# loganmcbroom/Flan

Measured on AMD Instinct MI355X. Metric: PV analysis+resynthesis frames/sec (2048-win, hop 512, 48 kHz) at 1/2/4/8 GPU, higher is better.
Workload: dtype f32; 1 GPU; 8 ch x 60 s x 48 kHz uniform noise per GPU, convert_to_PV(2048,512,dft 2048) -> convert_to_audio round trip; channels_per_gpu=8, parallelism=channel-shard x1

## Files before the change

### flan_amd/__init__.py

```python
import ctypes as C
import os

import numpy as np

_HERE = os.path.dirname(os.path.abspath(__file__))
LIB_PATH = os.environ.get("FLAN_AMD_LIB") or os.path.join(_HERE, "libflanhip.so")

OK, ERR_INVALID_ARG, ERR_UNSUPPORTED, ERR_HIP, ERR_CANCELLED, ERR_NO_DEVICE = 0, -1, -2, -3, -4, -5


class FlanHipError(RuntimeError):
    def __init__(self, code, message):
        super().__init__("flanhip error %d: %s" % (code, message))
        self.code = code


if not os.path.exists(LIB_PATH):
    raise ImportError("flan_amd/libflanhip.so is missing: build it with `python flan_amd/build.py` "
                      "(hipcc --offload-arch=gfx950); there is no fallback path")

lib = C.CDLL(LIB_PATH)

_f32p = np.ctypeslib.ndpointer(np.float32, flags="C_CONTIGUOUS")
_vp, _i64, _i32, _f32 = C.c_void_p, C.c_int64, C.c_int, C.c_float
# ... 13 lines not shown
    "flanhip_download": (C.c_int, [_vp, _vp, C.c_size_t]),
    "flanhip_touch_pages": (C.c_int, [_vp, C.c_size_t]),
    "flanhip_host_workers": (C.c_int, []),
    "flanhip_parallel_for": (C.c_int, [C.c_int, _vp, _vp]),
    "flanhip_stream_create": (C.c_int, [C.POINTER(_vp)]),
    "flanhip_stream_destroy": (C.c_int, [_vp]),
    "flanhip_host_malloc": (C.c_int, [C.POINTER(_vp), C.c_size_t]),
    "flanhip_host_free": (C.c_int, [_vp]),
    "flanhip_memcpy_h2d": (C.c_int, [_vp, _vp, C.c_size_t, _vp]),
    "flanhip_memcpy_d2h": (C.c_int, [_vp, _vp, C.c_size_t, _vp]),
    "flanhip_memset": (C.c_int, [_vp, _i32, C.c_size_t, _vp]),
    "flanhip_stream_synchronize": (C.c_int, [_vp]),
    "flanhip_wait_cancellable": (C.c_int, [_vp, _vp]),
    "flanhip_wait_cancellable_fn": (C.c_int, [_vp, _vp, _vp]),
    "flanhip_analyze": (C.c_int, [_vp, _i64, _i64, _f32, _i32, _i32, _i32, _vp, C.POINTER(_i64), _vp]),
    "flanhip_analyze_dev": (C.c_int, [_vp, _i64, _i64, _f32, _i32, _i32, _i32, _vp, _vp]),
    "flanhip_synthesize": (C.c_int, [_vp, _i64, _i64, _i32, _f32, _f32, _i32, _vp, C.POINTER(_i32), _vp]),
    "flanhip_synthesize_workspace_bytes": (C.c_size_t, [_i64, _i64, _i32, _f32, _f32, _i32]),
    "flanhip_synthesize_dev": (C.c_int, [_vp, _i64, _i64, _i32, _f32, _f32, _i32, _vp, _vp, _vp, _vp]),
    "flanhip_analyze_dev_fused": (C.c_int, [_vp, _i64, _i64, _f32, _i32, _i32, _i32, _vp, _vp, _vp]),
    "flanhip_synthesize_dev_fused": (C.c_int, [_vp, _i64, _i64, _i32, _f32, _f32, _i32, _vp, _vp, _vp, _vp]),
    "flanhip_synthesize_dev_stages": (C.c_int, [_vp, _i64, _i64, _i32, _f32, _f32, _i32, _vp, _vp, _vp, _i32, _i32, _vp]),
    "flanhip_debug_option": (None, [_i32, _i32]),
    "flanhip_debug_kernel_scratch_bytes": (_i32, [_i32]),
    "flanhip_modify_time": (C.c_int, [_vp, _i64, _i64, _i32, _f32, _i32, _vp, _i64, _vp, _vp]),
    "flanhip_modify_time_dev": (C.c_int, [_vp, _i64, _i64, _i32, _f32, _i32, _vp, _i64, _vp, _vp]),
    "flanhip_modify_time_dev_fused": (C.c_int, [_vp, _i64, _i64, _i32, _f32, _f32, _vp, _i64, _vp, _i32, _vp, _vp]),
    "flanhip_synthesize_dev_fused_checked": (C.c_int, [_vp, _i64, _i64, _i32, _f32, _f32, _i32, _vp, _vp, _vp, _vp]),
    "flanhip_stretch_map_dev": (C.c_int, [_vp, _i64, _i32, _f32, _i32, _vp, _vp]),
    "flanhip_stretch_map_const_dev": (C.c_int, [_f32, _vp, _i64, _i32, _f32, _i32, _vp, _vp]),
    "flanhip_fill_dev": (C.c_int, [_vp, _i64, _f32, _vp]),
    "flanhip_modify_frequency": (C.c_int, [_vp, _i64, _i64, _i32, _f32, _vp, _vp, _vp, _vp]),
    "flanhip_modify_frequency_dev": (C.c_int, [_vp, _i64, _i64, _i32, _f32, _vp, _vp, _vp, _vp]),
    "flanhip_modify_time_interp_dev": (C.c_int, [_vp, _i64, _i64, _i32, _f32, _i32, _vp, _i64, _i32, _vp, _vp]),
    "flanhip_modify_time_interp_dev_fused": (C.c_int, [_vp, _i64, _i64, _i32, _f32, _f32, _vp, _i64, _i32, _vp, _i32, _vp, _vp]),
    "flanhip_modify_frequency_interp_dev": (C.c_int, [_vp, _i64, _i64, _i32, _f32, _vp, _vp, _i32, _vp, _vp]),
    "flanhip_repitch_interp_dev": (C.c_int, [_vp, _i64, _i64, _i32, _f32, _vp, _i32, _vp, _vp]),
    "flanhip_repitch_map_dev": (C.c_int, [_vp, _i64, _i64, _i32, _f32, _vp, _vp, _vp]),
    "flanhip_repitch_dev": (C.c_int, [_vp, _i64, _i64, _i32, _f32, _vp, _vp, _vp]),
    "flanhip_shape_affine": (C.c_int, [_vp, _i64, _i64, _i32, _f32, _f32, _f32, _f32, _f32, _i32, _vp, _vp]),
    "flanhip_shape_affine_dev": (C.c_int, [_vp, _i64, _i64, _i32, _f32, _f32, _f32, _f32, _f32, _i32, _vp, _vp]),
    "flanhip_shape_table_dev": (C.c_int, [_vp, _vp, _i64, _i64, _i32, _f32, _i32, _vp, _vp]),
    "flanhip_replace_amplitudes_dev": (C.c_int, [_vp, _i64, _i64, _i32, _vp, _i64, _i64, _i32, _vp, _f32, _vp, _vp]),
    "flanhip_subtract_amplitudes_dev": (C.c_int, [_vp, _i64, _i64, _i32, _vp, _i64, _i64, _i32, _vp, _f32, _vp, _vp]),
    "flanhip_resonate_out_frames": (_i64, [_i64, _f32, _f32, _i32]),
    "flanhip_resonate_dev": (C.c_int, [_vp, _i64, _i64, _i32, _f32, _i32, _i64, _vp, _f32, _vp, _vp]),
# ... 442 lines not shown


def analyze_dev(d_audio, ch, n, sample_rate, window, hop, dft, d_out, stream=None):
    check(lib.flanhip_analyze_dev(_dp(d_audio), ch, n, sample_rate, window, hop, dft, _dp(d_out), _vp(stream or 0)))


def analyze_dev_fused(d_audio, ch, n, sample_rate, window, hop, dft, d_out, d_ws, stream=None):
    check(lib.flanhip_analyze_dev_fused(_dp(d_audio), ch, n, sample_rate, window, hop, dft, _dp(d_out), _dp(d_ws), _vp(stream or 0)))


def synthesize_dev_fused(d_pv, ch, F, bins, sample_rate, analysis_rate, window, d_out, d_ws, d_nan=None, stream=None):
    check(lib.flanhip_synthesize_dev_fused(_dp(d_pv), ch, F, bins, sample_rate, analysis_rate, window, _dp(d_out), _dp(d_ws),
                                           _dp(d_nan), _vp(stream or 0)))


def synthesize_dev_stages(d_pv, ch, F, bins, sample_rate, analysis_rate, window, d_out, d_ws, d_nan, presummed, stages, stream=None):
    check(lib.flanhip_synthesize_dev_stages(_dp(d_pv), ch, F, bins, sample_rate, analysis_rate, window, _dp(d_out), _dp(d_ws),
                                            _dp(d_nan), presummed, stages, _vp(stream or 0)))


DEBUG_CHAIN_LEN, DEBUG_TARGET_CHAINS, DEBUG_FORCE_GENERIC, DEBUG_NO_FAST_DIV = 0, 1, 2, 3
DEBUG_ANA_VARIANT, DEBUG_SYN_VARIANT, DEBUG_ANA4096_OLD, DEBUG_SYN4096_OLD, DEBUG_RESAMPLE_DIRECT, DEBUG_FORCE_DIRECT, DEBUG_INLINE_FIXUP, DEBUG_WIDE_OFFSETS = 4, 5, 6, 7, 8, 9, 10, 11
_DEBUG_NAMES = {"chain_len": 0, "target_chains": 1, "force_generic": 2, "no_fast_div": 3, "ana_variant": 4, "syn_variant": 5,
                "ana4096_old": 6, "syn4096_old": 7, "resample_direct": 8, "force_direct": 9, "inline_fixup": 10, "wide_offsets": 11, "no_sub": 12}


class debug_options:

    def __init__(self, **kw):
        self.kw = {_DEBUG_NAMES[k]: int(v) for k, v in kw.items()}

    def __enter__(self):
        for k, v in self.kw.items():
            lib.flanhip_debug_option(k, v)
        return self

    def __exit__(self, *exc):
        for k in self.kw:
            lib.flanhip_debug_option(k, 0)
        return False


def synthesize_workspace_bytes(ch, F, bins, sample_rate, analysis_rate, window):
    return int(lib.flanhip_synthesize_workspace_bytes(ch, F, bins, sample_rate, analysis_rate, window))


def synthesize_dev(d_pv, ch, F, bins, sample_rate, analysis_rate, window, d_out, d_ws, d_nan=None, stream=None):
# ... 101 lines not shown
```

### flan_amd/csrc/conversions.hip

```cpp
#include "flanhip_internal.h"
#include <atomic>
#include <memory>
#include "pv_kernels.h"
#include "pv_kernels_fast.h"
#include <type_traits>
#include "pv_kernels_v2.h"
#include "pv_kernels_v3.h"
#include "pv_kernels_eo.h"
#include "pv_kernels_any.h"
#include "pv_kernels_mr.h"
#include "pv_kernels_bs.h"
#include "pv_kernels_big.h"
#include "team_launch.h"
#include "sub_launch.h"
#include <algorithm>
#include <cstdlib>

namespace flanhip {


static constexpr int kMaxAnyDft = 1 << 20;
static bool fft_size( int dft ) { return is_pow2( dft ) && dft >= 32 && dft <= 8192; }
static int mr_blocks_per_cu( const MrPlan & pl, int W )
	{
// ... 342 lines not shown
	const bool n_ok = n >= 2 && n < ( int64_t( 1 ) << 31 ) - 8192;
	route_pow2( r, dft, n_ok && sub_shape( dft, W, hop ),
		n_ok && ( dft == 2048 || ( dft == 4096 && !debug_options().ana11_old ) || v3_size( dft ) ) && hop <= 65536 && !force_generic() );
	return r;
	}
static Route synthesis_route( int dft, int W, int hop )
	{
	Route r = size_route( dft, W, hop );
	r.min_len = r.family == Family::any ? 1 : std::max( ( W + hop - 1 ) / hop - 1, 1 );
	if( r.family != Family::generic ) return r;
	const bool sub = sub_shape( dft, W, hop );
	r.kind = sub ? 0 : synth_fast_kind( dft, W, hop );
	route_pow2( r, dft, sub, r.kind != 0 );
	return r;
	}

static int self_carry_group( const Route & syn, const SynthLayout & lay )
	{
	if( syn.family != Family::sub && syn.family != Family::fast ) return 0;
	if( syn.family == Family::fast && lay.dft == 4096 && debug_options().ana11_old ) return 0;
	return lay.chains_per_channel < 128 ? 0 : syn.block_group;
	}
static int synth_layout_routed( int64_t ch, int64_t F, int bins, float sr, float ar, int W, SynthLayout * o, Route * route );
int synth_layout( int64_t ch, int64_t F, int bins, float sr, float ar, int W, SynthLayout * o ) { Route r; return synth_layout_routed( ch, F, bins, sr, ar, W, o, &r ); }

static int launch_group_scan( const SynthParams & p, hipStream_t s )
	{
	if( p.groups_per_channel <= 512 ) hipLaunchKernelGGL( ( k_phase_scan2<16, true> ), dim3( (unsigned) ( ( p.num_bins + 31 ) / 32 ), (unsigned) p.num_channels ), dim3( 512 ), 0, s, p );
	else hipLaunchKernelGGL( ( k_phase_scan2<32, true> ), dim3( (unsigned) ( ( p.num_bins + 15 ) / 16 ), (unsigned) p.num_channels ), dim3( 512 ), 0, s, p );
	FLANHIP_CHECK( hipGetLastError() );
	return FLANHIP_OK;
	}
static int launch_group_sums( bool sums_too, int gsize, const SynthParams & p, double * gs, hipStream_t s )
	{
	const dim3 grid( (unsigned) ( ( p.num_bins + 255 ) / 256 ), (unsigned) p.groups_per_channel, (unsigned) p.num_channels );
	auto kern = sums_too ? ( gsize == 32 ? k_sums_and_groups<32> : gsize == 16 ? k_sums_and_groups<16> : gsize == 8 ? k_sums_and_groups<8> : k_sums_and_groups<4> )
		: ( gsize == 32 ? k_group_sums<32> : gsize == 16 ? k_group_sums<16> : gsize == 8 ? k_group_sums<8> : k_group_sums<4> );
	hipLaunchKernelGGL( kern, grid, dim3( 256 ), 0, s, p, gs );
	FLANHIP_CHECK( hipGetLastError() );
	return FLANHIP_OK;
	}
template<bool B> using bool_c = std::integral_constant<bool, B>;
template<int I> using int_c = std::integral_constant<int, I>;
template<typename F> static auto mr_kernel( const MrPlan & pl, F f )
	{
	return !mr_pingpong( pl.C ) ? f( bool_c<false>{}, bool_c<true>{} ) : mr_plan_is_big( pl ) ? f( bool_c<true>{}, bool_c<true>{} ) : f( bool_c<true>{}, bool_c<false>{} );
	}
template<typename F> static auto bs_kernel( const BsPlan & pl, int W, F f )
	{
	return !bs_pingpong( pl.M ) ? f( bool_c<false>{}, bool_c<false>{} ) : bs_hoist( pl, W ) ? f( bool_c<true>{}, bool_c<true>{} ) : f( bool_c<true>{}, bool_c<false>{} );
	}
template<int MIXED, typename F> static auto big_kernel_q( int bq, F f ) { return bq > 4 ? f( int_c<8>{}, int_c<MIXED>{} ) : bq > 2 ? f( int_c<4>{}, int_c<MIXED>{} ) : f( int_c<2>{}, int_c<MIXED>{} ); }
template<typename F> static auto big_kernel( const BigPlan & pl, F f )
	{
	const int bq = ( pl.C2 + MR_THREADS - 1 ) / MR_THREADS;
	return pl.mixed == 2 ? big_kernel_q<2>( bq, f ) : pl.mixed ? big_kernel_q<1>( bq, f ) : big_kernel_q<0>( bq, f );
	}

static int launch_analyze_body( const float * d_audio, int64_t ch, int64_t n, float sr, int W, int hop, int dft, flanhip_MF * d_out, void * d_fused_ws, hipStream_t s, bool * left_group_sums, int * epoch );

int launch_analyze( const float * d_audio, int64_t ch, int64_t n, float sr, int W, int hop, int dft, flanhip_MF * d_out, void * d_fused_ws, hipStream_t s )
	{
	bool left_group_sums = false;
	int epoch = 0;
	if( d_fused_ws ) note_workspace_producer( d_fused_ws, 0 );
	const int rc = launch_analyze_body( d_audio, ch, n, sr, W, hop, dft, d_out, d_fused_ws, s, &left_group_sums, &epoch );
	if( !rc && d_fused_ws && left_group_sums ) note_workspace_producer( d_fused_ws, 1, epoch );
	return rc;
	}

static int launch_analyze_body( const float * d_audio, int64_t ch, int64_t n, float sr, int W, int hop, int dft, flanhip_MF * d_out, void * d_fused_ws, hipStream_t s, bool * left_group_sums, int * epoch )
	{
	FLANHIP_REQUIRE( d_audio && d_out, FLANHIP_ERR_INVALID_ARG, "null buffer" );
	FLANHIP_REQUIRE( ch > 0 && n >= 0 && W >= 2 && hop >= 1 && sr > 0.0f, FLANHIP_ERR_INVALID_ARG, "bad sizes" );
	FLANHIP_REQUIRE( W <= dft, FLANHIP_ERR_INVALID_ARG, "window_size larger than dft_size" );
	FLANHIP_REQUIRE( dft_size_ok( dft ), FLANHIP_ERR_UNSUPPORTED, "dft_size must be even, at least 4 and at most 2^20" );
	if( int rc = require_device() ) return rc;
	const Route r = analysis_route( dft, W, hop, n );
	std::shared_ptr<const PlanRef> plan_ref;
	if( int rc = get_plan( W, dft, &plan_ref ) ) return rc;
	const Plan * plan = &plan_ref->plan;

	AnalyzeParams p{};
	p.audio = d_audio; p.out = reinterpret_cast<MF*>( d_out );
	p.window = plan->d_window; p.tw = plan->d_tw; p.tw2 = plan->d_tw2; p.dump = plan->d_dump;
	p.n = n; p.F = n / hop + 1;
	p.num_channels = int( ch ); p.window_size = W; p.hop = hop;
	p.L = choose_chain_length( ch, p.F, r.min_len, r.target_chains, r.block_group );
	p.chains_per_channel = int( ( p.F + p.L - 1 ) / p.L );
	p.sample_rate = sr;
	p.analysis_rate = sr / hop;
	DivPlan dp;
	if( int rc = get_div_plan( p.analysis_rate, &dp ) ) return rc;
	p.ar_div = DivC{ dp.c, dp.rc, dp.exact };
	p.sums = nullptr; p.nan_out = nullptr; p.nan_epoch = 0;
	p.cancel = thread_cancel_word( s );
	bool kernel_sums = r.family != Family::any && r.family != Family::big && ( r.family != Family::mr || mr_pingpong( r.mr.C ) ) && ( r.family != Family::bs || bs_pingpong( r.bs.M ) );
	SynthLayout fused_lay{};
	if( d_fused_ws )
		{
		SynthLayout & lay = fused_lay;
		Route syn;
		if( int rc = synth_layout_routed( ch, p.F, dft / 2 + 1, sr, p.analysis_rate, W, &lay, &syn ) ) return rc;
		p.nan_epoch = next_epoch();
		*epoch = p.nan_epoch;
		if( kernel_sums && lay.L >= p.L + 8 && int64_t( p.chains_per_channel ) * ch <= r.target_chains ) kernel_sums = false;
		if( kernel_sums )
			{
			p.L = lay.L;
			p.chains_per_channel = lay.chains_per_channel;
			p.sums = reinterpret_cast<double*>( d_fused_ws );
			p.nan_out = ws_at<int>( d_fused_ws, lay.carry_bytes + lay.head_bytes );
			}
		const bool groups_too = ( r.family == Family::fast || r.family == Family::sub ) && hop <= W && kernel_sums && self_carry_group( syn, lay ) != 0;
		p.group_sums = groups_too ? ws_at<double>( d_fused_ws, lay.group_offset ) : nullptr;
		p.groups_per_channel = lay.groups_per_channel;
		*left_group_sums = groups_too;
		}
	auto prepass_on_behalf = [&]() -> int
		{
		if( !d_fused_ws || kernel_sums ) return FLANHIP_OK;
		SynthParams q{};
		q.pv = reinterpret_cast<const MF*>( d_out );
		q.carry = reinterpret_cast<double*>( d_fused_ws );
		q.F = p.F; q.num_channels = int( ch ); q.num_bins = dft / 2 + 1;
		q.L = fused_lay.L; q.chains_per_channel = fused_lay.chains_per_channel;
		q.analysis_rate = p.analysis_rate; q.ar_div = p.ar_div;
		q.nan_words = ws_at<int>( d_fused_ws, fused_lay.carry_bytes + fused_lay.head_bytes );
		q.nan_epoch = p.nan_epoch;
		const int64_t chains = int64_t( q.chains_per_channel ) * ch;
		hipLaunchKernelGGL( k_phase_sums2, dim3( (unsigned) chains, (unsigned) ( ( q.num_bins + 255 ) / 256 ) ), dim3( 256 ), 0, s, q );
		FLANHIP_CHECK( hipGetLastError() );
		return FLANHIP_OK;
		};

	const int64_t chains = int64_t( p.chains_per_channel ) * ch;
	int rc = FLANHIP_ERR_UNSUPPORTED;
	switch( r.family )
		{
		case Family::team: rc = run_analyze_team( p, *plan, dft, s ); break;
// ... 167 lines not shown
	p.analysis_rate = ar;
	p.window_scale = 2.67f / ( lay.dft * W / lay.hop );
	DivPlan dp;
	if( int rc = get_div_plan( ar, &dp ) ) return rc;
	p.ar_div = DivC{ dp.c, dp.rc, dp.exact };
	p.dump = ws_at<float>( d_ws, lay.carry_bytes + lay.head_bytes + 512 );
	p.nan_in = ( presummed == 1 || presummed == 2 ) ? ws_at<const int>( d_ws, lay.carry_bytes + lay.head_bytes ) : nullptr;
	p.skip_words = presummed == 2 ? p.nan_in : nullptr;
	p.carry_in = d_carry_in; p.total_out = d_total_out; p.total_only = prepass_only ? 1 : 0;
	p.cancel = thread_cancel_word( s );
	const int fix_hook = debug_options().inline_fixup;
	const bool self_fix = lay.fix_offset != 0 && !prepass_only && ( stage_mask & 0xF ) == 0xF && fix_hook != 2
		&& ( fix_hook == 1 || lay.L >= ( lay.head_len + lay.hop - 1 ) / lay.hop + 3 );
	if( self_fix )
		{
		p.fix_state = ws_at<int>( d_ws, lay.fix_offset );
		p.tail = ws_at<float>( d_ws, lay.tail_offset );
		p.fix_tag = int( ( unsigned( next_epoch() ) & 0x1FFFFFFFu ) << 2 );
		}

	const int64_t chains = int64_t( p.chains_per_channel ) * ch;
	FLANHIP_REQUIRE( chains < ( int64_t( 1 ) << 31 ), FLANHIP_ERR_UNSUPPORTED, "too many chains for one launch" );
	const int stages = prepass_only ? 3 : ( stage_mask & 0xF );
	int noted_epoch = 0;
	const int gsize = self_carry_group( r, lay );
	const bool self_carry = presummed == 1 && !prepass_only && !d_carry_in && !d_total_out && debug_options().syn_variant != 2
		&& gsize != 0 && workspace_producer( d_ws, &noted_epoch ) == 1;
	if( self_carry )
		{
		p.expect_epoch = noted_epoch;
		p.group_sums = ws_at<const double>( d_ws, lay.group_offset );
		p.groups_per_channel = lay.groups_per_channel;
		const bool scan_groups = p.groups_per_channel > 40;
		p.group_carry = scan_groups ? ws_at<double>( d_ws, lay.group_offset + lay.group_bytes ) : nullptr;
		if( scan_groups && ( stages & 2 ) ) { if( int rc = launch_group_scan( p, s ) ) return rc; }
		}
	const bool group_kernel = !self_carry && gsize != 0 && stages == 0xF && !prepass_only && !d_carry_in && !d_total_out && debug_options().syn_variant != 2 && presummed != 3;
	const bool sums_in_group_kernel = group_kernel && presummed != 1;
	if( ( stages & 1 ) && presummed != 1 && presummed != 3 && !sums_in_group_kernel )
		{
		hipLaunchKernelGGL( k_phase_sums2, dim3( (unsigned) chains, (unsigned) ( ( bins + 255 ) / 256 ) ), dim3( 256 ), 0, s, p );
		FLANHIP_CHECK( hipGetLastError() );
		}
	if( group_kernel )
		{
		double * gs = ws_at<double>( d_ws, lay.group_offset );
		p.groups_per_channel = lay.groups_per_channel;
		FLANHIP_REQUIRE( lay.groups_per_channel <= 65535 && ch <= 65535, FLANHIP_ERR_UNSUPPORTED, "too many groups / channels for one launch" );
		if( int rc = launch_group_sums( sums_in_group_kernel, gsize, p, gs, s ) ) return rc;
		p.group_sums = gs;
		const bool scan_groups = p.groups_per_channel > 40;
		p.group_carry = scan_groups ? ws_at<double>( d_ws, lay.group_offset + lay.group_bytes ) : nullptr;
		if( scan_groups ) { if( int rc = launch_group_scan( p, s ) ) return rc; }
		}
	if( ( stages & 2 ) && !self_carry && !group_kernel )
		{
		const int64_t cols = ch * bins;
		const bool flat = p.chains_per_channel <= 64 && ( bins >= 2049 || cols >= 65536 ) && !d_carry_in && !d_total_out && !prepass_only;
		if( flat && p.chains_per_channel <= 32 ) hipLaunchKernelGGL( k_phase_scan_flat<32>, dim3( (unsigned) ( ( bins + 255 ) / 256 ), (unsigned) ch ), dim3( 256 ), 0, s, p );
		else if( flat ) hipLaunchKernelGGL( k_phase_scan_flat<64>, dim3( (unsigned) ( ( bins + 255 ) / 256 ), (unsigned) ch ), dim3( 256 ), 0, s, p );
		else if( p.chains_per_channel <= 512 ) hipLaunchKernelGGL( k_phase_scan2<16>, dim3( (unsigned) ( ( bins + 31 ) / 32 ), (unsigned) ch ), dim3( 512 ), 0, s, p );
		else if( p.chains_per_channel <= 1024 ) hipLaunchKernelGGL( k_phase_scan2<32>, dim3( (unsigned) ( ( bins + 15 ) / 16 ), (unsigned) ch ), dim3( 512 ), 0, s, p );
		else hipLaunchKernelGGL( k_phase_scan2<64>, dim3( (unsigned) ( ( bins + 7 ) / 8 ), (unsigned) ch ), dim3( 512 ), 0, s, p );
		FLANHIP_CHECK( hipGetLastError() );
		}

	int rc = FLANHIP_ERR_UNSUPPORTED;
	if( !( stages & 4 ) ) rc = FLANHIP_OK;
	else switch( r.family )
		{
		case Family::any:
			{
			std::shared_ptr<const UnitRef> unit_ref;
			if( int rc2 = get_unit_circle( lay.dft, &unit_ref ) ) return rc2;
// ... 178 lines not shown
	{
	FLANHIP_REQUIRE( presummed >= 0 && presummed <= 2, FLANHIP_ERR_INVALID_ARG, "presummed: 0, 1 or 2" );
	return launch_synthesize( d_pv, ch, F, bins, sr, ar, W, d_out, d_ws, d_nan, presummed, (hipStream_t) stream, nullptr, nullptr, false, stages );
	}

void flanhip_debug_option( int which, int value )
	{
	DebugOptions & o = debug_options();
	switch( which )
		{
		case FLANHIP_DEBUG_CHAIN_LEN:       o.chain_len = value; break;
		case FLANHIP_DEBUG_TARGET_CHAINS:   o.target_chains = value; break;
		case FLANHIP_DEBUG_FORCE_GENERIC:   o.force_generic = value; break;
		case FLANHIP_DEBUG_NO_FAST_DIV:     o.no_fast_div = value; break;
		case FLANHIP_DEBUG_ANA_VARIANT:     o.ana_variant = value; break;
		case FLANHIP_DEBUG_SYN_VARIANT:     o.syn_variant = value; break;
		case FLANHIP_DEBUG_ANA4096_OLD:     o.ana11_old = value; break;
		case FLANHIP_DEBUG_SYN4096_OLD:     o.syn11_old = value; break;
		case FLANHIP_DEBUG_RESAMPLE_DIRECT: o.resample_direct = value; break;
		case FLANHIP_DEBUG_FORCE_DIRECT:    o.force_direct = value; break;
		case FLANHIP_DEBUG_INLINE_FIXUP:    o.inline_fixup = value; break;
		case FLANHIP_DEBUG_WIDE_OFFSETS:    o.wide_offsets = value; break;
		case FLANHIP_DEBUG_NO_SUB:          o.no_sub = value; break;
		default: break;
		}
	}
#ifdef FLANHIP_STAMPS
int flanhip_debug_read_stamps( unsigned long long * out16 )
	{
	FLANHIP_CHECK( hipDeviceSynchronize() );
	FLANHIP_CHECK( hipMemcpyFromSymbol( out16, HIP_SYMBOL( g_stamp_acc ), 16 * sizeof( unsigned long long ) ) );
	unsigned long long zero[16] = { 0 };
	FLANHIP_CHECK( hipMemcpyToSymbol( HIP_SYMBOL( g_stamp_acc ), zero, sizeof( zero ) ) );
	return FLANHIP_OK;
	}
int flanhip_debug_read_spans( unsigned long long * out8192 )
	{
	FLANHIP_CHECK( hipDeviceSynchronize() );
	FLANHIP_CHECK( hipMemcpyFromSymbol( out8192, HIP_SYMBOL( g_stamp_span ), 8192 * sizeof( unsigned long long ) ) );
	return FLANHIP_OK;
	}
#endif

size_t flanhip_synthesize_workspace_bytes( int64_t ch, int64_t F, int bins, float sr, float ar, int W )
	{
	SynthLayout lay;
	if( synth_layout( ch, F, bins, sr, ar, W, &lay ) ) return 0;
	return lay.total_bytes;
	}

int flanhip_synthesize_dev( const flanhip_MF * d_pv, int64_t ch, int64_t F, int bins, float sr, float ar, int W,
	float * d_out, void * d_ws, int * d_nan, void * stream )
	{
	return launch_synthesize( d_pv, ch, F, bins, sr, ar, W, d_out, d_ws, d_nan, false, (hipStream_t) stream );
	}

int flanhip_synthesize( const flanhip_MF * pv, int64_t ch, int64_t F, int bins, float sr, float ar, int W,
	float * out, int * nan_flag, volatile int * cancel )
	{
	FLANHIP_REQUIRE( pv && out, FLANHIP_ERR_INVALID_ARG, "null buffer" );
	SynthLayout lay;
	if( int rc = synth_layout( ch, F, bins, sr, ar, W, &lay ) ) return rc;
	if( int rc = require_device() ) return rc;
	if( cancelled( cancel ) ) return FLANHIP_ERR_CANCELLED;
	const size_t pv_bytes = sizeof( flanhip_MF ) * size_t( ch ) * F * bins;
// ... 20 lines not shown
```

### flan_amd/csrc/flanhip_internal.h

```cpp
#pragma once
#include <hip/hip_runtime.h>
#include <cstdarg>
#include <cstdint>
#include <cstdio>
#include <cmath>
#include <map>
#include <memory>
#include <mutex>
#include <tuple>
#include <vector>

#include "flanhip.h"
#include "cf_type.h"

namespace flanhip {

void set_error( const char * fmt, ... );

#define FLANHIP_CHECK( expr )                                                                         \
	do { hipError_t e_ = ( expr );                                                                    \
		if( e_ != hipSuccess ) {                                                                      \
			::flanhip::set_error( "%s failed: %s (%s:%d)", #expr, hipGetErrorString( e_ ), __FILE__, __LINE__ ); \
			return FLANHIP_ERR_HIP; } } while( 0 )

// ... 37 lines not shown
	};
inline int team_radix( int dft_size ) { return dft_size == 8192 ? 4 : dft_size == 16384 ? 8 : 0; }
struct TeamTableLayout { int tw1, tw3, twj, tws, two, total; };
inline TeamTableLayout team_table_layout( int R ) { TeamTableLayout l; l.tw1 = 0; l.tw3 = 240; l.twj = 1008; l.tws = l.twj + ( R - 1 ) * 512; l.two = l.tws + ( R / 2 ) * 512; l.total = l.two + 2 * R; return l; }
struct PlanRef { Plan plan; PlanRef() = default; PlanRef( const PlanRef & ) = delete; PlanRef & operator=( const PlanRef & ) = delete; ~PlanRef(); };
int get_plan( int window_size, int dft_size, std::shared_ptr<const PlanRef> * out );

struct DivPlan { float c, rc; int exact; };
int get_div_plan( float c, DivPlan * out );

int choose_chain_length( int64_t num_channels, int64_t num_frames, int min_len, int target_chains, int group = 1 );
struct DebugOptions
	{
	int chain_len = 0;
	int target_chains = 0;
	int force_generic = 0;
	int no_fast_div = 0;
	int ana_variant = 0, syn_variant = 0;
	int ana11_old = 0, syn11_old = 0;
	int resample_direct = 0;
	int wide_offsets = 0;
	int inline_fixup = 0;
	int no_sub = 0;
	int force_direct = 0;
	};
DebugOptions & debug_options();
bool force_generic();
int cu_count();

int launch_analyze( const float * d_audio, int64_t ch, int64_t n, float sr, int W, int hop, int dft, flanhip_MF * d_out, void * d_fused_ws, hipStream_t s );
int launch_synthesize( const flanhip_MF * d_pv, int64_t ch, int64_t F, int bins, float sr, float ar, int W, float * d_out,
	void * d_ws, int * d_nan, int presummed, hipStream_t s, const double * d_carry_in = nullptr, double * d_total_out = nullptr,
	bool prepass_only = false, int stage_mask = 0xF );

int next_epoch();

struct SynthLayout { int hop, dft, L, chains_per_channel, head_len, groups_per_channel; size_t carry_bytes, head_bytes, group_offset, group_bytes, total_bytes;
	size_t flags_offset;
	size_t fix_offset, tail_offset;
	bool any; size_t any_spec_offset, any_frames_offset;
	size_t mr_ring_offset;
	size_t bsg_offset;
	bool big; size_t big_out_offset, big_head_offset, big_ring_offset; };
void note_workspace_producer( const void * d_ws, int kind, int epoch = 0 );
int workspace_producer( const void * d_ws, int * epoch = nullptr );
int synth_layout( int64_t ch, int64_t F, int bins, float sr, float ar, int W, SynthLayout * out );
// ... 9 lines not shown
```

### flan_amd/csrc/pv_kernels.h

```cpp
#pragma once
#include <hip/hip_runtime.h>
#include <stdint.h>
#include "fft_device.h"
#include "pv_math.h"

namespace flanhip {

struct MF { float m, f; };


struct AnalyzeParams
	{
	const float * audio;
	MF * out;
	const float * window;
	const cf * tw;
	const cf * tw2;
	int64_t n;
	int64_t F;
	int num_channels;
	int window_size;
	int hop;
	int L;
	int chains_per_channel;
	float sample_rate;
	float analysis_rate;
	DivC ar_div;
	double * sums;
	int * nan_out;
	int nan_epoch;
	double * group_sums;
	int groups_per_channel;
	const int * cancel;
	float * dump;
	};

__device__ __forceinline__ int cancel_peek( const int * word )
	{
	return word ? __hip_atomic_load( word, __ATOMIC_RELAXED, __HIP_MEMORY_SCOPE_SYSTEM ) : 0;
	}
__device__ __forceinline__ bool cancel_seen( int peeked ) { return __builtin_amdgcn_readfirstlane( peeked ) != 0; }

__device__ __forceinline__ MF phase_vocode_bin( float re, float im, float & prev_phase, float bin_frequency, float expected_phase_diff,
	float analysis_rate, bool use_wrapping )
	{
	const float phase = atan2_fast( im, re );
	const float phase_diff = phase - prev_phase;
	prev_phase = phase;
	const float delta_phase = phase_diff - expected_phase_diff;
	const float wrapped = use_wrapping ? delta_phase - FLANHIP_PI2_F * round_half_away( div_pi2( delta_phase ) ) : delta_phase;
	const float delta_frequency = div_pi2( wrapped * analysis_rate );
	MF r;
	r.m = magnitude_scaled( re, im );
	r.f = bin_frequency + delta_frequency;
	return r;
	}

// ... 194 lines not shown
	int chains_per_channel;
	int head_len;
	int num_bins;
	float analysis_rate;
	float window_scale;
	DivC ar_div;
	const int * nan_in;
	float * dump;
	const double * carry_in;
	double * total_out;
	int total_only;
	int * nan_words;
	int nan_epoch;
	int expect_epoch;
	const int * skip_words;
	const int * cancel;
	const double * group_sums;
	int groups_per_channel;
	double * group_carry;
	int * fix_state;
	float * tail;
	int fix_tag;
	float * ring_ws;
	};


template<int LOG2C, int WAVES, int T = 1>
__global__ __launch_bounds__( 64 * WAVES * T ) void k_synthesize( SynthParams p )
	{
	constexpr int C = 1 << LOG2C;
	static_assert( T == 1 || WAVES == 1, "a team of several wavefronts owns its block" );
	constexpr int TEAM = 64 * T, NT = 64 * WAVES * T;
	constexpr int E = ( C + TEAM - 1 ) / TEAM;
	constexpr bool BIG = LOG2C >= 12 && T == 1;
	constexpr int UNR = BIG ? 2 : E + 1;
	extern __shared__ __attribute__((aligned(16))) unsigned char smem[];
	cf * s_tw = reinterpret_cast<cf*>( smem );
	const int W = p.window_size, hop = p.hop;
	const int wpad = ( W + 3 ) & ~3;
	float * s_win = reinterpret_cast<float*>( s_tw + ( BIG ? 0 : C ) );
	cf * s_buf_all = reinterpret_cast<cf*>( s_win + wpad );
	float * s_ring_all = reinterpret_cast<float*>( s_buf_all + WAVES * padded_len( C + 1 ) );
	double * s_ph_all = reinterpret_cast<double*>( s_ring_all + WAVES * wpad );

	const int tid = threadIdx.x, lane = T == 1 ? ( tid & 63 ) : tid, wave = T == 1 ? ( tid >> 6 ) : 0;
	__shared__ int s_cancel;
// ... 200 lines not shown
```

### flan_amd/csrc/pv_kernels_v2.h

```cpp
#pragma once
#include "pv_kernels_fast.h"

namespace flanhip {

struct V2Lds
	{
	static constexpr int C = 1024;
	static constexpr int TW1 = 0;
	static constexpr int TW3 = TW1 + 240;
	static constexpr int W2H = TW3 + 768;
	static constexpr int WIN = W2H + 512;
	static constexpr int KC = WIN + 1024;
	static constexpr int BUF = KC + 1024;
	static constexpr int BUF_LEN = C + C / 16 + 1;
	static constexpr size_t bytes( int waves ) { return size_t( BUF + waves * BUF_LEN ) * 8; }
	};


#ifdef FLANHIP_STAMPS
__device__ unsigned long long g_stamp_acc[16];
__device__ unsigned long long g_stamp_span[2 * 4096];
struct Stamps
	{
	unsigned long long last, acc[12], t_begin, r_begin;
// ... 46 lines not shown
			const unsigned w = blockIdx.x * ( blockDim.x >> 6 ) + ( threadIdx.x >> 6 );
			if( w < 4096 ) { g_stamp_span[2 * w] = r_begin; g_stamp_span[2 * w + 1] = r_end; }
			}
		}
#endif
	};
#else
struct Stamps
	{
	__device__ __forceinline__ void init() {}
	__device__ __forceinline__ void operator()( int ) const {}
	__device__ __forceinline__ void flush( int ) {}
	};
#endif


#ifndef FLANHIP_PUBLISH_DRAIN
#define FLANHIP_PUBLISH_DRAIN 1
#endif
__device__ __forceinline__ void publish_drain()
	{
	if constexpr( FLANHIP_PUBLISH_DRAIN != 0 ) asm volatile( "s_waitcnt vmcnt(0)" ::: "memory" );
	else asm volatile( "" ::: "memory" );
	}

template<int WAVES, bool SUMS, int NV, int ABL = 0>
__global__ __launch_bounds__( 64 * WAVES ) void k_analyze_v2( AnalyzeParams p, FastTables tb )
	{
	using L = V2Lds;
	constexpr int C = 1024, E = 16, H = 8, NT = 64 * WAVES;
	constexpr int NP = NV / 2;
	static_assert( NV == 2 || NV == 4 || NV == 8 || NV == 16, "1, 2, 4 or 8 pairs at a time" );
	typedef float VB __attribute__(( ext_vector_type( NV ) ));
	extern __shared__ __attribute__((aligned(16))) unsigned char smem[];
	cf * s = reinterpret_cast<cf*>( smem );
	const int tid = threadIdx.x, lane = tid & 63, wave = tid >> 6;
	const int W = p.window_size, hop = p.hop;
	const int cancel_word = cancel_peek( p.cancel );

	for( int i = tid; i < 240; i += NT ) s[L::TW1 + i] = tb.tw1[i];
	for( int i = tid; i < 768; i += NT ) s[L::TW3 + i] = tb.tw3[i];
	for( int i = tid; i < 512; i += NT ) { const cf w = tb.w2[i]; s[L::W2H + i] = mk( 0.5f * w.x, 0.5f * w.y ); }
		{
		float * win = reinterpret_cast<float*>( s + L::WIN );
		for( int i = tid; i < 2 * C; i += NT ) win[i] = ( i < W ) ? p.window[i] : 0.0f;
		v4f_t * kc = reinterpret_cast<v4f_t*>( s + L::KC );
// ... 310 lines not shown
				}
			const double vx = fold( sumx );
			if( lane == 0 ) { dst[C / 2] = vx; stage[C / 2] = vx; }
			}
		const bool any_bad = __any( bad );
		if( p.nan_out && lane == 0 && active )
			{
			if( chain == 0 ) { p.nan_out[2] = p.nan_epoch; p.nan_out[4] = p.nan_epoch; }
			if( any_bad ) p.nan_out[0] = p.nan_epoch;
			}
		if( p.group_sums )
			{
			__syncthreads();
			const int live = min( WAVES, p.chains_per_channel - group * WAVES );
			double * gdst = p.group_sums + ( int64_t( channel ) * groups + group ) * ( C + 1 );
			for( int bin = tid; bin <= C; bin += NT )
				{
				double run = 0.0;
				for( int w = 0; w < live; ++w )
					{
					const double v = run + reinterpret_cast<const double*>( s + L::BUF + w * L::BUF_LEN )[bin];
					run = ( __builtin_fabs( v ) < FLANHIP_FOLD_FAST_LIMIT ) ? fold_phase_fast( v ) : fold_phase_any( v );
					}
				gdst[bin] = run;
				}
			}
		}
	}

__device__ __forceinline__ void st_agent( cf * p, cf v )
	{
	unsigned long long bits; __builtin_memcpy( &bits, &v, 8 );
	__hip_atomic_store( reinterpret_cast<unsigned long long*>( p ), bits, __ATOMIC_RELAXED, __HIP_MEMORY_SCOPE_AGENT );
	}
__device__ __forceinline__ cf ld_agent( const cf * p )
	{
	const unsigned long long bits = __hip_atomic_load( reinterpret_cast<const unsigned long long*>( p ), __ATOMIC_RELAXED, __HIP_MEMORY_SCOPE_AGENT );
	cf v; __builtin_memcpy( &v, &bits, 8 );
	return v;
	}

struct V2LdsSyn
	{
	static constexpr int C = 1024;
	static constexpr int TW1 = 0;
	static constexpr int TW3 = TW1 + 240;
	static constexpr int W2S = TW3 + 768;
// ... 141 lines not shown
			{
			#pragma unroll
			for( int b = 0; b < NB; ++b ) run[b] = gs[int64_t( group ) * ( C + 1 ) + bins_of[b]];
			}
		if( active ) load_row( relf0 );
		if( !p.group_carry )
			{
			for( int g0 = 0; g0 < group; g0 += 16 )
				{
				double v[NB][16];
				#pragma unroll
				for( int b = 0; b < NB; ++b )
					{
					#pragma unroll
					for( int u = 0; u < 16; ++u ) v[b][u] = ( g0 + u < group ) ? gs[int64_t( g0 + u ) * ( C + 1 ) + bins_of[b]] : 0.0;
					}
				#pragma unroll
				for( int u = 0; u < 16; ++u )
					{
					#pragma unroll
					for( int b = 0; b < NB; ++b ) run[b] = fold( run[b] + v[b][u] );
					}
				}
			}
		#pragma unroll
		for( int w = 0; w < WAVES; ++w )
			{
			#pragma unroll
			for( int b = 0; b < NB; ++b )
				{
				if( has[b] ) reinterpret_cast<double*>( s + L::BUF + w * L::BUF_LEN )[bins_of[b]] = run[b];
				run[b] = fold( run[b] + vc[b][w] );
				}
			}
		if( tid == 0 && blockIdx.x == 0 )
			{
			if( p.nan_in && p.nan_flag && p.nan_in[0] == p.nan_in[2] && p.nan_in[2] != 0 ) atomicOr( p.nan_flag, 1 );
			if( p.expect_epoch && p.nan_in && p.nan_flag && p.nan_in[2] != p.expect_epoch ) atomicOr( p.nan_flag, 2 );
			if( p.skip_words ) const_cast<int*>( p.skip_words )[4] = 0;
			}
		__syncthreads();
		const double * mine = reinterpret_cast<const double*>( buf );
		#pragma unroll
		for( int q = 0; q < H; ++q ) { phk[q] = mine[lane + 64 * q]; phm[q] = mine[C - lane - 64 * q]; }
		phx = mine[C / 2];
		wave_sync();
// ... 277 lines not shown
```

### include/flanhip.h

```cpp
#ifndef FLANHIP_H
#define FLANHIP_H

#include <stddef.h>
#include <stdint.h>

#ifdef __cplusplus
extern "C" {
#endif

#define FLANHIP_OK                 0
#define FLANHIP_ERR_INVALID_ARG   -1
#define FLANHIP_ERR_UNSUPPORTED   -2
#define FLANHIP_ERR_HIP           -3
#define FLANHIP_ERR_CANCELLED     -4
#define FLANHIP_ERR_NO_DEVICE     -5

typedef struct flanhip_MF { float m; float f; } flanhip_MF;

int          flanhip_version(void);
const char * flanhip_last_error(void);
int          flanhip_device_count(void);
int          flanhip_set_device(int device);
int          flanhip_get_device(int * device);

// ... 42 lines not shown
                                 float sample_rate, float analysis_rate, int window_size,
                                 float * d_out, void * d_workspace, int * d_nan_flag, void * stream);
int flanhip_synthesize_dev_fused_checked(const flanhip_MF * d_pv, int64_t num_channels, int64_t num_pv_frames, int num_bins,
                                         float sample_rate, float analysis_rate, int window_size,
                                         float * d_out, void * d_workspace, int * d_nan_flag, void * stream);

int flanhip_synthesize_dev_stages(const flanhip_MF * d_pv, int64_t num_channels, int64_t num_pv_frames, int num_bins,
                                  float sample_rate, float analysis_rate, int window_size,
                                  float * d_out, void * d_workspace, int * d_nan_flag, int presummed, int stages, void * stream);

#define FLANHIP_DEBUG_CHAIN_LEN       0
#define FLANHIP_DEBUG_TARGET_CHAINS   1
#define FLANHIP_DEBUG_FORCE_GENERIC   2
#define FLANHIP_DEBUG_NO_FAST_DIV     3
#define FLANHIP_DEBUG_ANA_VARIANT     4
#define FLANHIP_DEBUG_SYN_VARIANT     5
#define FLANHIP_DEBUG_ANA4096_OLD     6
#define FLANHIP_DEBUG_SYN4096_OLD     7
#define FLANHIP_DEBUG_RESAMPLE_DIRECT 8
#define FLANHIP_DEBUG_FORCE_DIRECT    9
#define FLANHIP_DEBUG_INLINE_FIXUP   10
#define FLANHIP_DEBUG_WIDE_OFFSETS   11
#define FLANHIP_DEBUG_NO_SUB         12
void flanhip_debug_option(int which, int value);
int flanhip_debug_kernel_scratch_bytes(int which);

int flanhip_modify_time(const flanhip_MF * pv, int64_t num_channels, int64_t num_pv_frames, int num_bins,
                        float sample_rate, int hop, const float * mod_seconds,
                        int64_t out_frames, flanhip_MF * out, volatile int * cancel);
int flanhip_modify_time_dev(const flanhip_MF * d_pv, int64_t num_channels, int64_t num_pv_frames, int num_bins,
                            float sample_rate, int hop, const float * d_mod_seconds,
                            int64_t out_frames, flanhip_MF * d_out, void * stream);
int flanhip_modify_time_dev_fused(const flanhip_MF * d_pv, int64_t num_channels, int64_t num_pv_frames, int num_bins,
                                  float sample_rate, float analysis_rate, const float * d_mod, int64_t out_frames,
                                  flanhip_MF * d_out, int window_size, void * d_workspace, void * stream);
int flanhip_stretch_map_dev(float * d_factor, int64_t num_pv_frames, int num_bins, float sample_rate, int hop,
                            float * d_max, void * stream);
int flanhip_stretch_map_const_dev(float factor, float * d_map, int64_t num_pv_frames, int num_bins, float sample_rate, int hop,
                                  float * d_max, void * stream);
int flanhip_fill_dev(float * d_grid, int64_t count, float value, void * stream);

int flanhip_modify_frequency(const flanhip_MF * pv, int64_t num_channels, int64_t num_pv_frames, int num_bins,
                             float sample_rate, const float * mod_hz, const float * in_modified,
                             flanhip_MF * out, volatile int * cancel);
int flanhip_modify_frequency_dev(const flanhip_MF * d_pv, int64_t num_channels, int64_t num_pv_frames, int num_bins,
                                 float sample_rate, const float * d_mod_hz, const float * d_in_modified,
                                 flanhip_MF * d_out, void * stream);
// ... 152 lines not shown
```

Before: 167.6 million frames/s.

## Compute synthesis group carry prefix in analysis kernel via last-block ticket

When the analysis kernel writes per-group phase sums for a 2048-point fast route with few groups, it now takes an atomic ticket per channel slot. The last-arriving block computes the exclusive prefix of group sums and stores a finished group_carry buffer. Synthesis sees the new producer kind and reads the precomputed carries instead of scanning group sums itself. This moves serial prefix work out of each synthesis block, at the cost of atomics, fences and one block doing a serial tail in analysis.

```diff
diff --git a/flan_amd/__init__.py b/flan_amd/__init__.py
--- a/flan_amd/__init__.py
+++ b/flan_amd/__init__.py
@@ -59,6 +59,7 @@
     "flanhip_synthesize_dev_fused": (C.c_int, [_vp, _i64, _i64, _i32, _f32, _f32, _i32, _vp, _vp, _vp, _vp]),
     "flanhip_synthesize_dev_stages": (C.c_int, [_vp, _i64, _i64, _i32, _f32, _f32, _i32, _vp, _vp, _vp, _i32, _i32, _vp]),
     "flanhip_debug_option": (None, [_i32, _i32]),
+    "flanhip_debug_group_carry_range": (C.c_int, [_i64, _i64, _i32, _f32, _f32, _i32, C.POINTER(C.c_size_t), C.POINTER(_i32)]),
     "flanhip_debug_kernel_scratch_bytes": (_i32, [_i32]),
     "flanhip_modify_time": (C.c_int, [_vp, _i64, _i64, _i32, _f32, _i32, _vp, _i64, _vp, _vp]),
     "flanhip_modify_time_dev": (C.c_int, [_vp, _i64, _i64, _i32, _f32, _i32, _vp, _i64, _vp, _vp]),
@@ -547,7 +548,7 @@
 DEBUG_CHAIN_LEN, DEBUG_TARGET_CHAINS, DEBUG_FORCE_GENERIC, DEBUG_NO_FAST_DIV = 0, 1, 2, 3
 DEBUG_ANA_VARIANT, DEBUG_SYN_VARIANT, DEBUG_ANA4096_OLD, DEBUG_SYN4096_OLD, DEBUG_RESAMPLE_DIRECT, DEBUG_FORCE_DIRECT, DEBUG_INLINE_FIXUP, DEBUG_WIDE_OFFSETS = 4, 5, 6, 7, 8, 9, 10, 11
 _DEBUG_NAMES = {"chain_len": 0, "target_chains": 1, "force_generic": 2, "no_fast_div": 3, "ana_variant": 4, "syn_variant": 5,
-                "ana4096_old": 6, "syn4096_old": 7, "resample_direct": 8, "force_direct": 9, "inline_fixup": 10, "wide_offsets": 11, "no_sub": 12}
+                "ana4096_old": 6, "syn4096_old": 7, "resample_direct": 8, "force_direct": 9, "inline_fixup": 10, "wide_offsets": 11, "no_sub": 12, "group_carry": 13}
 
 
 class debug_options:
diff --git a/flan_amd/csrc/conversions.hip b/flan_amd/csrc/conversions.hip
--- a/flan_amd/csrc/conversions.hip
+++ b/flan_amd/csrc/conversions.hip
@@ -388,6 +388,9 @@
 	return lay.chains_per_channel < 128 ? 0 : syn.block_group;
 	}
 static int synth_layout_routed( int64_t ch, int64_t F, int bins, float sr, float ar, int W, SynthLayout * o, Route * route );
+constexpr int kSelfSumGroups = 40;
+constexpr size_t kTicketOffset = 64;
+constexpr int kTicketWords = 56;
 int synth_layout( int64_t ch, int64_t F, int bins, float sr, float ar, int W, SynthLayout * o ) { Route r; return synth_layout_routed( ch, F, bins, sr, ar, W, o, &r ); }
 
 static int launch_group_scan( const SynthParams & p, hipStream_t s )
@@ -423,19 +426,19 @@
 	return pl.mixed == 2 ? big_kernel_q<2>( bq, f ) : pl.mixed ? big_kernel_q<1>( bq, f ) : big_kernel_q<0>( bq, f );
 	}
 
-static int launch_analyze_body( const float * d_audio, int64_t ch, int64_t n, float sr, int W, int hop, int dft, flanhip_MF * d_out, void * d_fused_ws, hipStream_t s, bool * left_group_sums, int * epoch );
+static int launch_analyze_body( const float * d_audio, int64_t ch, int64_t n, float sr, int W, int hop, int dft, flanhip_MF * d_out, void * d_fused_ws, hipStream_t s, int * left_kind, int * epoch );
 
 int launch_analyze( const float * d_audio, int64_t ch, int64_t n, float sr, int W, int hop, int dft, flanhip_MF * d_out, void * d_fused_ws, hipStream_t s )
 	{
-	bool left_group_sums = false;
+	int left_kind = 0;
 	int epoch = 0;
 	if( d_fused_ws ) note_workspace_producer( d_fused_ws, 0 );
-	const int rc = launch_analyze_body( d_audio, ch, n, sr, W, hop, dft, d_out, d_fused_ws, s, &left_group_sums, &epoch );
-	if( !rc && d_fused_ws && left_group_sums ) note_workspace_producer( d_fused_ws, 1, epoch );
+	const int rc = launch_analyze_body( d_audio, ch, n, sr, W, hop, dft, d_out, d_fused_ws, s, &left_kind, &epoch );
+	if( !rc && d_fused_ws && left_kind ) note_workspace_producer( d_fused_ws, left_kind, epoch );
 	return rc;
 	}
 
-static int launch_analyze_body( const float * d_audio, int64_t ch, int64_t n, float sr, int W, int hop, int dft, flanhip_MF * d_out, void * d_fused_ws, hipStream_t s, bool * left_group_sums, int * epoch )
+static int launch_analyze_body( const float * d_audio, int64_t ch, int64_t n, float sr, int W, int hop, int dft, flanhip_MF * d_out, void * d_fused_ws, hipStream_t s, int * left_kind, int * epoch )
 	{
 	FLANHIP_REQUIRE( d_audio && d_out, FLANHIP_ERR_INVALID_ARG, "null buffer" );
 	FLANHIP_REQUIRE( ch > 0 && n >= 0 && W >= 2 && hop >= 1 && sr > 0.0f, FLANHIP_ERR_INVALID_ARG, "bad sizes" );
@@ -481,7 +484,14 @@
 		const bool groups_too = ( r.family == Family::fast || r.family == Family::sub ) && hop <= W && kernel_sums && self_carry_group( syn, lay ) != 0;
 		p.group_sums = groups_too ? ws_at<double>( d_fused_ws, lay.group_offset ) : nullptr;
 		p.groups_per_channel = lay.groups_per_channel;
-		*left_group_sums = groups_too;
+		*left_kind = groups_too ? 1 : 0;
+		if( groups_too && r.family == Family::fast && syn.family == Family::fast && dft == 2048 && lay.groups_per_channel <= kSelfSumGroups && debug_options().group_carry == 0 )
+			{
+			p.group_carry = ws_at<double>( d_fused_ws, lay.group_offset + lay.group_bytes );
+			p.tickets = ws_at<unsigned long long>( d_fused_ws, lay.carry_bytes + lay.head_bytes + kTicketOffset );
+			p.ticket_words = kTicketWords;
+			*left_kind = 2;
+			}
 		}
 	auto prepass_on_behalf = [&]() -> int
 		{
@@ -695,17 +705,20 @@
 	const int64_t chains = int64_t( p.chains_per_channel ) * ch;
 	FLANHIP_REQUIRE( chains < ( int64_t( 1 ) << 31 ), FLANHIP_ERR_UNSUPPORTED, "too many chains for one launch" );
 	const int stages = prepass_only ? 3 : ( stage_mask & 0xF );
-	int noted_epoch = 0;
+	int noted_epoch = 0, noted_kind = 0;
 	const int gsize = self_carry_group( r, lay );
 	const bool self_carry = presummed == 1 && !prepass_only && !d_carry_in && !d_total_out && debug_options().syn_variant != 2
-		&& gsize != 0 && workspace_producer( d_ws, &noted_epoch ) == 1;
+		&& gsize != 0 && ( noted_kind = workspace_producer( d_ws, &noted_epoch ) ) != 0;
 	if( self_carry )
 		{
 		p.expect_epoch = noted_epoch;
 		p.group_sums = ws_at<const double>( d_ws, lay.group_offset );
 		p.groups_per_channel = lay.groups_per_channel;
-		const bool scan_groups = p.groups_per_channel > 40;
-		p.group_carry = scan_groups ? ws_at<double>( d_ws, lay.group_offset + lay.group_bytes ) : nullptr;
+		const bool scan_groups = p.groups_per_channel > kSelfSumGroups;
+		const int carry_hook = debug_options().group_carry;
+		const bool finished = !scan_groups && noted_kind == 2 && carry_hook == 0;
+		p.group_carry = scan_groups || finished ? ws_at<double>( d_ws, lay.group_offset + lay.group_bytes ) : nullptr;
+		if( !scan_groups && carry_hook == 2 && r.family == Family::fast && lay.dft == 2048 ) p.prefix_out = ws_at<double>( d_ws, lay.group_offset + lay.group_bytes );
 		if( scan_groups && ( stages & 2 ) ) { if( int rc = launch_group_scan( p, s ) ) return rc; }
 		}
 	const bool group_kernel = !self_carry && gsize != 0 && stages == 0xF && !prepass_only && !d_carry_in && !d_total_out && debug_options().syn_variant != 2 && presummed != 3;
@@ -722,7 +735,7 @@
 		FLANHIP_REQUIRE( lay.groups_per_channel <= 65535 && ch <= 65535, FLANHIP_ERR_UNSUPPORTED, "too many groups / channels for one launch" );
 		if( int rc = launch_group_sums( sums_in_group_kernel, gsize, p, gs, s ) ) return rc;
 		p.group_sums = gs;
-		const bool scan_groups = p.groups_per_channel > 40;
+		const bool scan_groups = p.groups_per_channel > kSelfSumGroups;
 		p.group_carry = scan_groups ? ws_at<double>( d_ws, lay.group_offset + lay.group_bytes ) : nullptr;
 		if( scan_groups ) { if( int rc = launch_group_scan( p, s ) ) return rc; }
 		}
@@ -947,6 +960,7 @@
 		case FLANHIP_DEBUG_INLINE_FIXUP:    o.inline_fixup = value; break;
 		case FLANHIP_DEBUG_WIDE_OFFSETS:    o.wide_offsets = value; break;
 		case FLANHIP_DEBUG_NO_SUB:          o.no_sub = value; break;
+		case FLANHIP_DEBUG_GROUP_CARRY:     o.group_carry = value; break;
 		default: break;
 		}
 	}
@@ -966,6 +980,16 @@
 	return FLANHIP_OK;
 	}
 #endif
+
+int flanhip_debug_group_carry_range( int64_t ch, int64_t F, int bins, float sr, float ar, int W, size_t * offset, int * groups_per_channel )
+	{
+	FLANHIP_REQUIRE( offset && groups_per_channel, FLANHIP_ERR_INVALID_ARG, "null result" );
+	SynthLayout lay;
+	if( int rc = synth_layout( ch, F, bins, sr, ar, W, &lay ) ) return rc;
+	*offset = lay.group_offset + lay.group_bytes;
+	*groups_per_channel = lay.groups_per_channel;
+	return FLANHIP_OK;
+	}
 
 size_t flanhip_synthesize_workspace_bytes( int64_t ch, int64_t F, int bins, float sr, float ar, int W )
 	{
diff --git a/flan_amd/csrc/flanhip_internal.h b/flan_amd/csrc/flanhip_internal.h
--- a/flan_amd/csrc/flanhip_internal.h
+++ b/flan_amd/csrc/flanhip_internal.h
@@ -83,6 +83,7 @@
 	int wide_offsets = 0;
 	int inline_fixup = 0;
 	int no_sub = 0;
+	int group_carry = 0;
 	int force_direct = 0;
 	};
 DebugOptions & debug_options();
diff --git a/flan_amd/csrc/pv_kernels.h b/flan_amd/csrc/pv_kernels.h
--- a/flan_amd/csrc/pv_kernels.h
+++ b/flan_amd/csrc/pv_kernels.h
@@ -33,6 +33,9 @@
 	int groups_per_channel;
 	const int * cancel;
 	float * dump;
+	double * group_carry;
+	unsigned long long * tickets;
+	int ticket_words;
 	};
 
 __device__ __forceinline__ int cancel_peek( const int * word )
@@ -273,6 +276,7 @@
 	float * tail;
 	int fix_tag;
 	float * ring_ws;
+	double * prefix_out;
 	};
 
 
diff --git a/flan_amd/csrc/pv_kernels_v2.h b/flan_amd/csrc/pv_kernels_v2.h
--- a/flan_amd/csrc/pv_kernels_v2.h
+++ b/flan_amd/csrc/pv_kernels_v2.h
@@ -92,6 +92,28 @@
 	{
 	if constexpr( FLANHIP_PUBLISH_DRAIN != 0 ) asm volatile( "s_waitcnt vmcnt(0)" ::: "memory" );
 	else asm volatile( "" ::: "memory" );
+	}
+
+__device__ __forceinline__ void st_agent_f64( double * p, double v )
+	{
+	unsigned long long bits; __builtin_memcpy( &bits, &v, 8 );
+	__hip_atomic_store( reinterpret_cast<unsigned long long*>( p ), bits, __ATOMIC_RELAXED, __HIP_MEMORY_SCOPE_AGENT );
+	}
+__device__ __forceinline__ double ld_agent_f64( const double * p )
+	{
+	const unsigned long long bits = __hip_atomic_load( reinterpret_cast<const unsigned long long*>( p ), __ATOMIC_RELAXED, __HIP_MEMORY_SCOPE_AGENT );
+	double v; __builtin_memcpy( &v, &bits, 8 );
+	return v;
+	}
+__device__ __forceinline__ unsigned ticket_take( unsigned long long * word, unsigned epoch )
+	{
+	unsigned long long seen = __hip_atomic_load( word, __ATOMIC_RELAXED, __HIP_MEMORY_SCOPE_AGENT );
+	for( ;; )
+		{
+		const unsigned before = unsigned( seen >> 32 ) == epoch ? unsigned( seen ) : 0u;
+		const unsigned long long want = ( static_cast<unsigned long long>( epoch ) << 32 ) | ( before + 1u );
+		if( __hip_atomic_compare_exchange_strong( word, &seen, want, __ATOMIC_RELAXED, __ATOMIC_RELAXED, __HIP_MEMORY_SCOPE_AGENT ) ) return before;
+		}
 	}
 
 template<int WAVES, bool SUMS, int NV, int ABL = 0>
@@ -448,7 +470,64 @@
 					const double v = run + reinterpret_cast<const double*>( s + L::BUF + w * L::BUF_LEN )[bin];
 					run = ( __builtin_fabs( v ) < FLANHIP_FOLD_FAST_LIMIT ) ? fold_phase_fast( v ) : fold_phase_any( v );
 					}
-				gdst[bin] = run;
+				if( p.group_carry ) st_agent_f64( gdst + bin, run ); else gdst[bin] = run;
+				}
+			if( p.group_carry )
+				{
+				asm volatile( "s_waitcnt vmcnt(0)" ::: "memory" );
+				__syncthreads();
+				int * const last_flag = reinterpret_cast<int*>( s + L::TW1 );
+				const int T = min( p.num_channels, p.ticket_words );
+				const int tk = channel % T;
+				if( tid == 0 )
+					{
+					__builtin_amdgcn_fence( __ATOMIC_RELEASE, "agent" );
+					asm volatile( "s_waitcnt vmcnt(0)" ::: "memory" );
+					const unsigned arrivals = unsigned( groups ) * unsigned( ( p.num_channels - tk + T - 1 ) / T );
+					const bool last = ticket_take( p.tickets + tk, unsigned( p.nan_epoch ) ) + 1u == arrivals;
+					if( last ) { __builtin_amdgcn_fence( __ATOMIC_ACQUIRE, "agent" ); asm volatile( "s_waitcnt vmcnt(0)" ::: "memory" ); }
+					*last_flag = last ? 1 : 0;
+					}
+				__syncthreads();
+				if( *last_flag )
+					{
+					auto fold = []( double r )
+						{
+						return ( __builtin_fabs( r ) < FLANHIP_FOLD_FAST_LIMIT ) ? fold_phase_loop( r ) : fold_phase_any( r );
+						};
+					constexpr int NB = ( C + NT ) / NT, U = 8;
+					for( int c = tk; c < p.num_channels; c += T )
+						{
+						const double * gs = p.group_sums + int64_t( c ) * groups * ( C + 1 );
+						double * gc = p.group_carry + int64_t( c ) * groups * ( C + 1 );
+						double run[NB];
+						#pragma unroll
+						for( int b = 0; b < NB; ++b ) run[b] = 0.0;
+						for( int g0 = 0; g0 < groups; g0 += U )
+							{
+							double v[NB][U];
+							#pragma unroll
+							for( int b = 0; b < NB; ++b )
+								{
+								const int bin = tid + NT * b;
+								#pragma unroll
+								for( int u = 0; u < U; ++u ) v[b][u] = ( g0 + u < groups && bin <= C ) ? ld_agent_f64( gs + int64_t( g0 + u ) * ( C + 1 ) + bin ) : 0.0;
+								}
+							#pragma unroll
+							for( int u = 0; u < U; ++u )
+								{
+								const int g = g0 + u;
+								#pragma unroll
+								for( int b = 0; b < NB; ++b )
+									{
+									const int bin = tid + NT * b;
+									if( g < groups && bin <= C ) gc[int64_t( g ) * ( C + 1 ) + bin] = ( g & 15 ) ? fold( run[b] + 0.0 ) : run[b];
+									run[b] = fold( run[b] + v[b][u] );
+									}
+								}
+							}
+						}
+					}
 				}
 			}
 		}
@@ -636,6 +715,11 @@
 					for( int b = 0; b < NB; ++b ) run[b] = fold( run[b] + v[b][u] );
 					}
 				}
+			if( p.prefix_out )
+				{
+				#pragma unroll
+				for( int b = 0; b < NB; ++b ) if( has[b] ) p.prefix_out[( int64_t( channel ) * groups + group ) * ( C + 1 ) + bins_of[b]] = run[b];
+				}
 			}
 		#pragma unroll
 		for( int w = 0; w < WAVES; ++w )
diff --git a/include/flanhip.h b/include/flanhip.h
--- a/include/flanhip.h
+++ b/include/flanhip.h
@@ -88,7 +88,10 @@
 #define FLANHIP_DEBUG_INLINE_FIXUP   10
 #define FLANHIP_DEBUG_WIDE_OFFSETS   11
 #define FLANHIP_DEBUG_NO_SUB         12
+#define FLANHIP_DEBUG_GROUP_CARRY    13
 void flanhip_debug_option(int which, int value);
+int flanhip_debug_group_carry_range(int64_t num_channels, int64_t num_pv_frames, int num_bins, float sample_rate, float analysis_rate,
+                                    int window_size, size_t * offset, int * groups_per_channel);
 int flanhip_debug_kernel_scratch_bytes(int which);
 
 int flanhip_modify_time(const flanhip_MF * pv, int64_t num_channels, int64_t num_pv_frames, int num_bins,
```

Result: slower. 150.3 million frames/s (-10.3%).
